# hillerlab/GenomeAlignmentTools

Measured on AMD Instinct MI355X. Metric: aligned Gbases scored/sec, chainNet -rescore hg38-mm10, 1/2/4/8 MI355X, higher is better.
Workload: dtype int64; 1 GPU; chainNet -rescore end to end (bin/chainNet), C5 whole genome; generator=gac_synth c5, seed=1234, scale=1, t_seqs=455, q_seqs=66, chains=4999999, blocks=116489921, input_aligned_bases=4660467906, netted_chains=4701362, netted_aligned_bases=4397257687, parallelism=chromosome-side shards x1

## Files before the change

### genomealignmenttools_amd/csrc/host/gac_net.c

```c
#define _GNU_SOURCE
#include "gac_host.h"

#include <immintrin.h>
#include <sched.h>
#include <stdint.h>
#include <sys/mman.h>
#include <pthread.h>
#include <stdatomic.h>
#include <math.h>
#include <stdarg.h>
#include <stdio.h>
#include <time.h>
#include <stdlib.h>
#include <string.h>

#define BIGNUM 0x3fffffff

typedef struct ngap ngap;
typedef struct nfill nfill;

struct ngap {
    int start, end, o_start, o_end;
    nfill *fill_head;
    nfill **fills;
    int n_fills;
    ngap *next;
    nfill *pfill;
    int32_t pidx;
};

struct nfill {
    int start, end, o_start, o_end;
    int32_t chain;
    int32_t ali;
    ngap **gaps;
    int n_gaps;
    int32_t full;
    nfill *next;
    int64_t ord;
    ngap *pgap;
    int32_t pidx, level;
    int32_t wb0, wn;
};

typedef struct nchrom {
    const char *name;
    int size;
    ngap *root;
    int32_t sroot;
    int32_t height;
} nchrom;

typedef struct arena {
    char **blocks;
    size_t *sizes;
    size_t n, cap, used, bsize;
} arena;

#define ARENA_BLOCK ((size_t)32 << 20)
#define ARENA_ALIGN ((size_t)2 << 20)

static char *arena_map(size_t bs) {
    size_t len = bs + ARENA_ALIGN;
    char *m = mmap(NULL, len, PROT_READ | PROT_WRITE, MAP_PRIVATE | MAP_ANONYMOUS, -1, 0);
    if (m == MAP_FAILED) {
        fprintf(stderr, "gac_net: out of memory mapping %zu bytes\n", bs);
        abort();
    }
    char *p = (char *)(((uintptr_t)m + ARENA_ALIGN - 1) & ~(uintptr_t)(ARENA_ALIGN - 1));
    if (p > m)
        munmap(m, (size_t)(p - m));
    if (p + bs < m + len)
        munmap(p + bs, (size_t)(m + len - (p + bs)));
#ifdef MADV_HUGEPAGE
    madvise(p, bs, MADV_HUGEPAGE);
#endif
    return p;
}

static void *arena_alloc(arena *a, size_t sz) {
    sz = (sz + 15) & ~(size_t)15;
    if (a->n == 0 || a->used + sz > a->bsize) {
        if (a->n == a->cap) {
            a->cap = a->cap ? a->cap * 2 : 64;
            a->blocks = realloc(a->blocks, a->cap * sizeof(char *));
            a->sizes = realloc(a->sizes, a->cap * sizeof(size_t));
        }
        size_t bs = sz > ARENA_BLOCK ? (sz + ARENA_ALIGN - 1) & ~(ARENA_ALIGN - 1) : ARENA_BLOCK;
        a->blocks[a->n] = arena_map(bs);
        a->sizes[a->n++] = bs;
        a->bsize = bs;
        a->used = 0;
    }
    char *p = a->blocks[a->n - 1] + a->used;
    a->used += sz;
    if (a->used + 512 <= a->bsize)
        __builtin_prefetch(p + sz + 384, 1, 3);
    return p;
}

static int g_free_madv = -1;

static void arena_free(arena *a) {
    for (size_t i = 0; i < a->n && g_free_madv == 1; ++i)
        madvise(a->blocks[i], a->sizes[i], MADV_DONTNEED);
    for (size_t i = 0; i < a->n; ++i)
        munmap(a->blocks[i], a->sizes[i]);
    free(a->blocks);
    free(a->sizes);
    memset(a, 0, sizeof(*a));
}

typedef struct nwork {
    arena ar;
    struct sleaf *lf;
    int32_t lf_n, lf_cap, lf_free;
    struct snode *in;
    int32_t in_n, in_cap, in_free;
    struct sitem *q, *it, *cmb;
    int64_t q_n, q_cap, it_n, it_cap, cmb_cap;
    int32_t *rs, *re, *ros, *roe, *ro;
    int64_t r_cap;
    struct nfill **sf;
    int64_t sf_cap;
    char pad[64];
} nwork;

struct gac_net {
    gac_net_input in;
    gac_net_opts opt;
    int64_t n_netted;
    nchrom *chroms[2];
    int32_t n_chroms[2];
    nwork *w;
    int n_w;
    int64_t *chain_ali;
    nfill **order[2];
    int64_t n_order[2];
    int64_t *pord[2];
    int pord_ok[2];
    pthread_mutex_t pord_mu;
    int64_t *top[2];
    int64_t n_top[2];
    int32_t *nlen[2];
    int sides;
    int lookahead;
    atomic_int free_next;
// ... 370 lines not shown
        sleaf *L = &w->lf[y];
        for (int k = lo; k < hi; ++k) {
            L->start[k - lo] = cb[k].start;
            L->end[k - lo] = cb[k].end;
            L->gap[k - lo] = cb[k].gap;
        }
        L->n = hi - lo;
        if (p > 0) {
            L->prev = prev;
            w->lf[prev].next = y;
        }
        prev = y;
        nk[p] = spkey(cb[lo].start, cb[lo].end);
        nc[p] = y;
    }
    w->lf[prev].next = after;
    if (after >= 0)
        w->lf[after].prev = prev;
    sp_inner_insert(w, c, pn, pi, H - 1, nk + 1, nc + 1, parts - 1);
    free(nk);
    free(nc);
}

static ngap *gap_new(nwork *n, int s, int e, int os, int oe) {
    ngap *g = arena_alloc(&n->ar, sizeof(ngap));
    g->start = s;
    g->end = e;
    g->o_start = os;
    g->o_end = oe;
    return g;
}

static int strictly_inside(const gac_net *n, int min_start, int max_end, int start, int end) {
    return min_start < start && start + n->opt.min_space <= end && end < max_end;
}

static void it_push(nwork *w, int32_t s, int32_t e, ngap *g) {
    if (w->it_n == w->it_cap) {
        w->it_cap = w->it_cap ? w->it_cap * 2 : 1024;
        w->it = realloc(w->it, (size_t)w->it_cap * sizeof(sitem));
    }
    w->it[w->it_n++] = (sitem){s, e, g};
}


static void add_chain_side(const gac_net *net, nwork *n, nchrom *c, int32_t chain, int nb,
                           const int32_t *s, const int32_t *e, const int32_t *gos,
                           const int32_t *goe, const int32_t *os, int inv, int oflip, int cstart,
                           int cend, int boff) {
    sp_query(n, c, cstart, cend, s, e, nb);
    const int64_t nsp = n->q_n;
    for (int64_t si = 0; si < nsp; ++si)
        __builtin_prefetch(&n->q[si].gap->fill_head, 1);
    int k = 0;
    for (int64_t si = 0; si < nsp; ++si) {
        const int sstart = n->q[si].start, send = n->q[si].end;
        ngap *sgap = n->q[si].gap;
        while (k + 1 < nb && s[k + 1] <= sstart)
            ++k;
        int start = BIGNUM, end = -BIGNUM, zero = 0;
        int fs = BIGNUM, fe = -BIGNUM, omin = BIGNUM, omax = -BIGNUM;
        int wfirst = -1, wlast = -2;
        int64_t ali = 0;
        for (int b = k; b < nb; ++b) {
            const int b0 = s[b], b1 = e[b];
            if (b1 <= sstart)
                continue;
            if (b0 >= send)
                break;
            if (wfirst < 0)
                wfirst = b;
            wlast = b;
            const int cs = b0 < sstart ? sstart : b0, ce = b1 > send ? send : b1;
            if (start > cs)
                start = cs;
            if (end < ce)
                end = ce;
            ali += ce - cs;
            if (ce > cs) {
                const int o0 = inv ? os[b] + (b1 - ce) : os[b] + (cs - b0);
                const int o1 = inv ? os[b] + (b1 - cs) : os[b] + (ce - b0);
                if (fs > cs) fs = cs;
                if (fe < ce) fe = ce;
                if (omin > o0) omin = o0;
                if (omax < o1) omax = o1;
            } else {
                zero = 1;
            }
        }
        if (end < 0 || end - start < net->opt.min_fill)
            continue;
        nfill *f = arena_alloc(&n->ar, sizeof(nfill));
        f->start = start;
        f->end = end;
        f->chain = chain;
        f->ali = (int32_t)ali;
        if (zero) {
            fs = BIGNUM, fe = -BIGNUM, omin = BIGNUM, omax = -BIGNUM;
            for (int b = k; b < nb; ++b) {
                const int bs = s[b], be = e[b];
                if (be <= start)
                    continue;
                if (bs >= end)
                    break;
                const int cs = bs < start ? start : bs, ce = be > end ? end : be;
                const int o0 = inv ? os[b] + (be - ce) : os[b] + (cs - bs);
                const int o1 = inv ? os[b] + (be - cs) : os[b] + (ce - bs);
                if (fs > cs) fs = cs;
                if (fe < ce) fe = ce;
                if (omin > o0) omin = o0;
                if (omax < o1) omax = o1;
            }
        }
        {
            if (oflip >= 0) {
                const int t = omin;
                omin = oflip - omax;
                omax = oflip - t;
            }
            f->start = fs;
            f->end = fe;
            f->o_start = omin;
            f->o_end = omax;
            f->full = fs <= cstart && fe >= cend;
        }
        if (boff >= 0) {
            if (zero) {
                wfirst = k;
                while (wfirst < nb && e[wfirst] <= fs)
                    ++wfirst;
                wlast = wfirst - 1;
                while (wlast + 1 < nb && s[wlast + 1] < fe)
                    ++wlast;
            }
            f->wb0 = boff + (wfirst < 0 ? 0 : wfirst);
            f->wn = wfirst < 0 ? 0 : wlast - wfirst + 1;
        }
        nfill *h = __atomic_load_n(&sgap->fill_head, __ATOMIC_RELAXED);
        do
            f->next = h;
        while (!__atomic_compare_exchange_n(&sgap->fill_head, &h, f, 1, __ATOMIC_RELEASE,
                                            __ATOMIC_RELAXED));
        n->it_n = 0;
        if (start - sstart >= net->opt.min_space)
            it_push(n, sstart, start, sgap);
        const int64_t g0 = n->it_n;
        for (int b = k; b + 1 < nb; ++b) {
            int gs = e[b], ge = s[b + 1];
            if (ge >= send)
                break;
            if (strictly_inside(net, sstart, send, gs, ge))
                it_push(n, gs, ge, gap_new(n, gs, ge, gos[b], goe[b]));
        }
        f->n_gaps = (int)(n->it_n - g0);
        f->gaps = f->n_gaps ? arena_alloc(&n->ar, f->n_gaps * sizeof(ngap *)) : NULL;
        for (int i = 0; i < f->n_gaps; ++i)
            f->gaps[i] = n->it[g0 + i].gap;
        if (send - end >= net->opt.min_space)
            it_push(n, end, send, sgap);
        sp_replace(n, c, sstart, send, n->it, (int)n->it_n);
    }
}

static void ensure_rev(nwork *n, int64_t nb) {
    if (nb > n->r_cap) {
        n->r_cap = nb * 2;
        n->rs = realloc(n->rs, n->r_cap * 4);
        n->re = realloc(n->re, n->r_cap * 4);
        n->ros = realloc(n->ros, n->r_cap * 4);
        n->roe = realloc(n->roe, n->r_cap * 4);
        n->ro = realloc(n->ro, n->r_cap * 4);
    }
}

static int is_haplotype(const char *name) {
    return strstr(name, "_hap") != NULL || strstr(name, "_alt") != NULL;
}

typedef struct crec {
    int64_t boff;
// ... 105 lines not shown
}

static int cmp_fill(const void *a, const void *b) {
    const nfill *x = *(nfill *const *)a, *y = *(nfill *const *)b;
    return (x->start > y->start) - (x->start < y->start);
}

typedef struct fin_ctx {
    gac_net *n;
    nwork *w;
    int side;
    nfill **ord;
    int64_t n_ord, cap;
} fin_ctx;

static void finish_gap(fin_ctx *x, ngap *g);

static void finish_fill(fin_ctx *x, nfill *f) {
    if (x->n_ord == x->cap) {
        x->cap = x->cap ? x->cap * 2 : 256;
        x->ord = realloc(x->ord, (size_t)x->cap * sizeof(nfill *));
    }
    x->ord[x->n_ord++] = f;
    for (int i = 0; i < f->n_gaps; ++i) {
        f->gaps[i]->pfill = f;
        f->gaps[i]->pidx = i;
    }
    for (int i = 0; i < f->n_gaps; ++i)
        finish_gap(x, f->gaps[i]);
}

static void sort_gap_fills(nwork *w, ngap *g) {
    if (!g->fill_head) {
        g->n_fills = 0;
        g->fills = NULL;
        return;
    }
    int cnt = 0;
    for (nfill *f = g->fill_head; f; f = f->next) {
        if (cnt == w->sf_cap) {
            w->sf_cap = w->sf_cap ? 2 * w->sf_cap : 4096;
            w->sf = realloc(w->sf, (size_t)w->sf_cap * sizeof(nfill *));
        }
        w->sf[cnt++] = f;
    }
    g->n_fills = cnt;
    g->fills = arena_alloc(&w->ar, cnt * sizeof(nfill *));
    copy_fill(g->fills, w->sf, cnt);
    const int32_t level = g->pfill ? g->pfill->level + 1 : 0;
    if (cnt <= 16) {
        for (int i = 1; i < cnt; ++i) {
            nfill *v = g->fills[i];
            int j = i - 1;
            while (j >= 0 && g->fills[j]->start > v->start) {
                g->fills[j + 1] = g->fills[j];
                --j;
            }
            g->fills[j + 1] = v;
        }
    } else {
        qsort(g->fills, g->n_fills, sizeof(nfill *), cmp_fill);
    }
    for (int i = 0; i < cnt; ++i) {
        g->fills[i]->pgap = g;
        g->fills[i]->pidx = i;
        g->fills[i]->level = level;
    }
}

static void finish_gap(fin_ctx *x, ngap *g) {
    sort_gap_fills(x->w, g);
    for (int i = 0; i < g->n_fills; ++i)
        finish_fill(x, g->fills[i]);
}

static void *free_worker(void *arg) {
    gac_net *n = arg;
    for (;;) {
        int i = atomic_fetch_add(&n->free_next, 1);
        if (i >= n->n_w)
            return NULL;
        nwork *w = &n->w[i];
        arena_free(&w->ar);
        free(w->lf);
        free(w->in);
        free(w->q);
        free(w->it);
        free(w->cmb);
        free(w->rs);
        free(w->re);
        free(w->ros);
        free(w->roe);
        free(w->ro);
        free(w->sf);
    }
}
// ... 156 lines not shown

typedef struct sk_item {
    nfill *f;
    ngap *g;
    int64_t cnt;
} sk_item;

typedef struct skel {
    sk_item *it;
    int64_t n, cap;
} skel;

static void sk_push(skel *k, nfill *f, ngap *g) {
    if (k->n == k->cap) {
        k->cap = k->cap ? k->cap * 2 : 256;
        k->it = realloc(k->it, (size_t)k->cap * sizeof(sk_item));
    }
    k->it[k->n++] = (sk_item){f, g, 0};
}

static void skel_fill(nwork *w, skel *k, nfill *f) {
    sk_push(k, f, NULL);
    for (int i = 0; i < f->n_gaps; ++i) {
        f->gaps[i]->pfill = f;
        f->gaps[i]->pidx = i;
    }
    for (int i = 0; i < f->n_gaps; ++i) {
        ngap *g = f->gaps[i];
        if (f->level < SKEL_DEPTH) {
            sort_gap_fills(w, g);
            for (int j = 0; j < g->n_fills; ++j)
                skel_fill(w, k, g->fills[j]);
        } else if (g->fill_head) {
            sk_push(k, NULL, g);
        } else {
            g->n_fills = 0;
            g->fills = NULL;
        }
    }
}

typedef struct ispan {
    nfill **src;
    int64_t pos, cnt;
    int side;
} ispan;

typedef struct splice_job {
    gac_net *n;
    ispan *sp;
    int64_t nspan;
    _Atomic int64_t next;
} splice_job;

static void *splice_thread(void *arg) {
    splice_job *J = arg;
    for (;;) {
        const int64_t a = atomic_fetch_add(&J->next, 4096);
        if (a >= J->nspan)
            return NULL;
// ... 17 lines not shown
    sk_item **gi;
    int64_t n_gi, per;
    fin_ctx *x;
    int64_t ntask;
    _Atomic int64_t next;
    _Atomic int wid;
} fin_job;

static void *fin_thread(void *arg) {
    fin_job *F = arg;
    gac_net *n = F->n;
    nwork *w = &n->w[atomic_fetch_add(&F->wid, 1)];
    if (F->phase == 0) {
        const int64_t nc = n->n_chroms[GAC_T] + (int64_t)n->n_chroms[GAC_Q];
        for (;;) {
            const int64_t k = atomic_fetch_add(&F->next, 1);
            if (k >= nc)
                break;
            const int side = k < n->n_chroms[GAC_T] ? GAC_T : GAC_Q;
            nchrom *c = &n->chroms[side][side == GAC_T ? k : k - n->n_chroms[GAC_T]];
            if (!c->root)
                continue;
            sort_gap_fills(w, c->root);
            for (int j = 0; j < c->root->n_fills; ++j)
                skel_fill(w, &F->sk[k], c->root->fills[j]);
        }
        return NULL;
    }
    for (;;) {
        const int64_t k = atomic_fetch_add(&F->next, 1);
        if (k >= F->ntask)
            break;
        fin_ctx *x = &F->x[k];
        x->n = n;
        x->w = w;
        const int64_t a = k * F->per, b = a + F->per < F->n_gi ? a + F->per : F->n_gi;
        for (int64_t i = a; i < b; ++i) {
            const int64_t before = x->n_ord;
            finish_gap(x, F->gi[i]->g);
            F->gi[i]->cnt = x->n_ord - before;
        }
    }
    return NULL;
}

typedef struct net_task {
    int side;
    int32_t chrom;
// ... 240 lines not shown
    }
    free(bin);
    int64_t *rw = calloc((size_t)nc + 1, 8), mx = 0;
    for (int64_t i = 0; i < rest; ++i) {
        const int cs = t->recs[B->m + i].s, ce = t->recs[B->m + i].e;
        const int64_t a = upper_bound32(cuts, nc, cs), b = upper_bound32(cuts, nc, ce > cs ? ce - 1 : cs);
        for (int64_t r = a; r <= b; ++r)
            rw[r] += chain_work_in(cs, ce, t->recs[B->m + i].nb, r ? cuts[r - 1] : 0,
                                   r < nc ? cuts[r] : size);
    }
    for (int32_t r = 0; r <= nc; ++r)
        mx = rw[r] > mx ? rw[r] : mx;
    free(rw);
    *pmax = mx;
    *ptot = tot;
    return nc + 1;
}

static double mono_s(void);

static void big_prefix(gac_net *n, nwork *w, big_net *B, int nthreads) {
    net_task *t = B->t;
    nchrom *c = &n->chroms[t->side][t->chrom];
    c->root = gap_new(w, 0, c->size, 0, 0);
    c->root->pidx = t->chrom;
    sp_init(w, c, 0, c->size, c->root);
    const int32_t want = 4 * nthreads;
    int32_t *cuts = malloc((size_t)want * 4);
    B->t_start = mono_s();
    int64_t m = t->n < 8 ? t->n : 8, done = 0;
    sitem *sp = NULL;
    int64_t nsp = 0;
    int32_t nreg = 1;
    double t_add = 0, t_cut = 0, t0 = mono_s();
    const double t_gather = t0 - B->t_start;
    for (;;) {
        double ta = mono_s();
        net_chains(n, w, t->side, t->recs + done, m - done, c, INT32_MIN, INT32_MAX);
        done = m;
        double tb = mono_s();
        t_add += tb - ta;
        B->m = m;
        free(sp);
        sp = sp_all(w, c, &nsp);
        int64_t mx, tot;
        nreg = place_cuts(n, B, sp, nsp, want, c->size, cuts, &mx, &tot);
        t_cut += mono_s() - tb;
        if (m >= t->n || mx * nthreads <= tot * 5 / 4 || m >= t->n / 4)
// ... 60 lines not shown
    net_task *task;
    int64_t ntask;
    big_net *big;
    int32_t nbig;
    region **rq;
    int64_t nrq;
    _Atomic int64_t next, rnext, rpub;
    pthread_mutex_t rmu;
    _Atomic int ready;
    _Atomic int wid;
    _Atomic int32_t bnext, bdone;
    int nthreads;
    double t0;
    double prefix_s;
} net_job;

static int region_cmp(const void *a, const void *b) {
    const region *x = *(region *const *)a, *y = *(region *const *)b;
    return (x->work < y->work) - (x->work > y->work);
}

static void net_small(gac_net *n, nwork *w, const net_task *t) {
    nchrom *c = &n->chroms[t->side][t->chrom];
    c->root = gap_new(w, 0, c->size, 0, 0);
    c->root->pidx = t->chrom;
    sp_init(w, c, 0, c->size, c->root);
    net_chains(n, w, t->side, t->recs, t->n, c, INT32_MIN, INT32_MAX);
}

static double mono_s(void) {
    struct timespec t;
    clock_gettime(CLOCK_MONOTONIC, &t);
    return t.tv_sec + 1e-9 * t.tv_nsec;
}

static void *net_thread(void *arg) {
    net_job *J = arg;
    const int id = atomic_fetch_add(&J->wid, 1);
    nwork *w = &J->n->w[id];
    for (;;) {
        const int32_t b = atomic_fetch_add(&J->bnext, 1);
        if (b >= J->nbig)
            break;
        big_prefix(J->n, w, &J->big[b], J->nthreads);
        big_net *B = &J->big[b];
        region **tmp = malloc((size_t)(B->n_reg ? B->n_reg : 1) * sizeof(region *));
        for (int32_t r = 0; r < B->n_reg; ++r)
            tmp[r] = &B->reg[r];
// ... 179 lines not shown
        return gac_fail(GAC_E_ARG, "gac_net_build_sides: bad side mask %d", sides);
    return net_build(in, opt, sides, NULL, NULL, out);
}

int gac_net_build_subset(const gac_net_input *in, const gac_net_opts *opt, const uint8_t *t_keep,
                         const uint8_t *q_keep, gac_net **out) {
    gac_clear_error();
    if (!in || !opt || !out || !t_keep || !q_keep)
        return gac_fail(GAC_E_ARG, "gac_net_build_subset: NULL argument");
    return net_build(in, opt, (1 << GAC_T) | (1 << GAC_Q), t_keep, q_keep, out);
}

static int net_build(const gac_net_input *in, const gac_net_opts *opt, int sides,
                     const uint8_t *t_keep, const uint8_t *q_keep, gac_net **out) {
    *out = NULL;
    gac_net *n = calloc(1, sizeof(*n));
    if (n)
        pthread_mutex_init(&n->pord_mu, NULL);
    n->in = *in;
    n->opt = *opt;
    n->sides = sides;
    n->n_w = gac_host_threads();
    n->w = calloc((size_t)n->n_w, sizeof(nwork));
    for (int k = 0; k < n->n_w; ++k) {
        n->w[k].lf_free = -1;
        n->w[k].in_free = -1;
    }
    struct timespec t_set0, t_set1;
    clock_gettime(CLOCK_MONOTONIC, &t_set0);
    double last = -1;
    int64_t i;
    for (i = 0; i < in->n_chains; ++i) {
        const double sc = in->score[i];
        if (last >= 0 && sc > last) {
            gac_net_free(n);
            return gac_fail(GAC_E_FORMAT, "input must be sorted in order of score");
        }
        last = sc;
        if (sc < opt->min_score)
            break;
        if (in->t_seq[i] < 0 || in->t_seq[i] >= in->n_tseq || in->q_seq[i] < 0 ||
            in->q_seq[i] >= in->n_qseq) {
            gac_net_free(n);
            return gac_fail(GAC_E_ARG, "chain %lld: sequence index out of range", (long long)i);
        }
    }
    const int64_t nn = i;
    int32_t nt = in->n_tseq, nq = in->n_qseq;
    int64_t *toff, *qoff;
// ... 132 lines not shown
            for (int64_t i = 0; i < F.sk[k].n; ++i)
                tot[side] += F.sk[k].it[i].g ? F.sk[k].it[i].cnt : 1;
        }
        for (int side = 0; side < 2; ++side) {
            n->order[side] = malloc((size_t)(tot[side] ? tot[side] : 1) * sizeof(nfill *));
            n->n_order[side] = 0;
        }
        int64_t nspan = 0;
        for (int64_t k = 0; k < nc; ++k)
            nspan += F.sk[k].n;
        splice_job SJ = {n, malloc((size_t)(nspan ? nspan : 1) * sizeof(ispan)), nspan, 0};
        for (int side = 0; side < 2; ++side) {
            n->top[side] = malloc((size_t)(nspan ? nspan : 1) * sizeof(int64_t));
            n->n_top[side] = 0;
        }
        {
            int64_t gidx = 0, used = 0, m = 0;
            for (int64_t k = 0; k < nc; ++k) {
                const int side = k < n->n_chroms[GAC_T] ? GAC_T : GAC_Q;
                for (int64_t i = 0; i < F.sk[k].n; ++i) {
                    sk_item *it = &F.sk[k].it[i];
                    if (!it->g) {
                        SJ.sp[m++] = (ispan){&it->f, n->n_order[side], 1, side};
                        if (it->f->level == 0)
                            n->top[side][n->n_top[side]++] = n->n_order[side];
                        ++n->n_order[side];
                        continue;
                    }
                    const fin_ctx *x = &F.x[gidx / F.per];
                    if (gidx % F.per == 0)
                        used = 0;
                    SJ.sp[m++] = (ispan){x->ord + used, n->n_order[side], it->cnt, side};
                    n->n_order[side] += it->cnt;
                    used += it->cnt;
                    ++gidx;
                }
            }
        }
        atomic_init(&SJ.next, 0);
        gac_run_threads(n->n_w, splice_thread, &SJ);
        free(SJ.sp);
        for (int64_t k = 0; k < nc; ++k)
            free(F.sk[k].it);
        for (int64_t k = 0; k < F.ntask; ++k)
            free(F.x[k].ord);
        free(F.sk);
        free(F.gi);
        struct timespec t_b;
        clock_gettime(CLOCK_MONOTONIC, &t_b);
        if (getenv("GAC_TIMING"))
            fprintf(stderr, "[gac_net_build] finishNet skeletons %.3f s, subtrees %.3f s, index %.3f s (%lld gap subtrees in %lld chunks)\n",
                    (t_a.tv_sec - t_fin0.tv_sec) + 1e-9 * (t_a.tv_nsec - t_fin0.tv_nsec),
                    (t_sp.tv_sec - t_a.tv_sec) + 1e-9 * (t_sp.tv_nsec - t_a.tv_nsec),
                    (t_b.tv_sec - t_sp.tv_sec) + 1e-9 * (t_b.tv_nsec - t_sp.tv_nsec), (long long)F.n_gi,
                    (long long)F.ntask);
        free(F.x);
    }
    clock_gettime(CLOCK_MONOTONIC, &t_fin1);
    if (getenv("GAC_TIMING")) {
        size_t sp_bytes = 0, ar_bytes = 0;
        for (int i = 0; i < n->n_w; ++i) {
            sp_bytes += (size_t)n->w[i].lf_cap * sizeof(sleaf) + (size_t)n->w[i].in_cap * sizeof(snode);
            for (size_t k = 0; k < n->w[i].ar.n; ++k)
                ar_bytes += n->w[i].ar.sizes[k];
        }
        fprintf(stderr, "[gac_net_build] finishNet %.3f s (space index %.0f MB, fill/gap arenas %.0f MB)\n",
                (t_fin1.tv_sec - t_fin0.tv_sec) + 1e-9 * (t_fin1.tv_nsec - t_fin0.tv_nsec),
                sp_bytes / 1e6, ar_bytes / 1e6);
    }
    space_release(n);
    for (int side = 0; side < 2; ++side) {
        const int32_t ns = side == GAC_T ? in->n_tseq : in->n_qseq;
        const char *const *nm = side == GAC_T ? in->t_names : in->q_names;
        n->nlen[side] = malloc((size_t)(ns > 0 ? ns : 1) * sizeof(int32_t));
        for (int32_t k = 0; k < ns; ++k)
            n->nlen[side][k] = (int32_t)strlen(nm[k]);
    }
    n->chain_ali = malloc((size_t)(in->n_chains ? in->n_chains : 1) * sizeof(int64_t));
    {
        ca_job A = {in, n->chain_ali, 0};
        atomic_init(&A.next, 0);
        gac_run_threads(gac_host_threads(), chain_ali_thread, &A);
    }
    *out = n;
    return GAC_OK;
}

int64_t gac_net_netted(const gac_net *n) { return n ? n->n_netted : -1; }

int64_t gac_net_fill_count(const gac_net *n, int side) {
    if (!n || (side != GAC_T && side != GAC_Q))
// ... 6 lines not shown
typedef struct gf_job {
    const gac_net *n;
    int side;
    int32_t *chain, *start, *end, *ali;
    uint8_t *flags;
    int64_t per;
    _Atomic int64_t next;
    int32_t *wb0, *wn;
    int64_t *po;
} gf_job;

static void *fills_thread(void *arg) {
    gf_job *J = arg;
    const gac_net *n = J->n;
    const int side = J->side;
    for (;;) {
        const int64_t a = atomic_fetch_add(&J->next, 1) * J->per;
        if (a >= n->n_order[side])
            break;
        const int64_t b = a + J->per < n->n_order[side] ? a + J->per : n->n_order[side];
        for (int64_t i = a; i < b; ++i) {
            const nfill *f = n->order[side][i];
            const int64_t c = f->chain;
            const int full = f->full;
            const int sz = full ? full_size(n, c) : f->ali;
            if (J->chain)
                J->chain[i] = (int32_t)c;
            if (J->start)
                J->start[i] = f->start;
            if (J->end)
                J->end[i] = f->end;
            if (J->ali)
                J->ali[i] = sz;
            if (J->flags)
                J->flags[i] = (uint8_t)(full ? 0 : 1);
            if (J->wb0)
                J->wb0[i] = f->wb0;
            if (J->wn)
                J->wn[i] = f->wn;
        }
    }
    return NULL;
}

static int64_t next_top_level(const gac_net *n, int side, int64_t i) {
    if (n->top[side]) {
        const int64_t *t = n->top[side];
        int64_t lo = 0, hi = n->n_top[side];
        while (lo < hi) {
            const int64_t mid = (lo + hi) >> 1;
            if (t[mid] < i)
                lo = mid + 1;
            else
                hi = mid;
        }
        return lo < n->n_top[side] ? t[lo] : n->n_order[side];
    }
    if (__atomic_load_n(&n->pord_ok[side], __ATOMIC_ACQUIRE)) {
        const int64_t *po = n->pord[side];
        while (i < n->n_order[side] && po[i] >= 0)
            ++i;
        return i;
    }
    while (i < n->n_order[side] && n->order[side][i]->pgap->pfill)
        ++i;
    return i;
}

static void *visible_thread(void *arg) {
    gf_job *J = arg;
    const gac_net *n = J->n;
    const int side = J->side;
    const int64_t nf = n->n_order[side];
    for (;;) {
        const int64_t r = atomic_fetch_add(&J->next, 1);
        if (r * J->per >= nf)
            break;
        const int64_t a = next_top_level(n, side, r * J->per);
        const int64_t b = next_top_level(n, side, (r + 1) * J->per < nf ? (r + 1) * J->per : nf);
        int64_t *po = J->po;
        for (int64_t i = a; i < b; ++i) {
            const nfill *pf = n->order[side][i]->pgap->pfill;
            if (po)
                po[i] = pf ? pf->ord : -1;
            const int sz = J->ali ? J->ali[i] : 0;
            if ((!pf || (J->flags[pf->ord] & 2)) && sz >= n->opt.min_fill)
                J->flags[i] |= 2;
        }
    }
    return NULL;
}

int gac_net_get_fills(const gac_net *n, int side, int32_t *chain, int32_t *start, int32_t *end,
                      int32_t *ali, uint8_t *flags) {
    if (!n || (side != GAC_T && side != GAC_Q))
        return gac_fail(GAC_E_ARG, "gac_net_get_fills: bad argument");
    if (!(n->sides & (1 << side)))
        return gac_fail(GAC_E_STATE, "gac_net_get_fills: side %d was not netted", side);
    const int nt = gac_host_threads();
    const int64_t nf = n->n_order[side];
    gf_job J = {n, side, chain, start, end, ali, flags, nf / (8 * (int64_t)nt) + 1, 0, NULL, NULL};
    atomic_init(&J.next, 0);
    const int64_t nrun = (nf + J.per - 1) / J.per;
    gac_mark("get_fills: fills");
    gac_run_threads(nt < nrun ? nt : (int)(nrun ? nrun : 1), fills_thread, &J);
// ... 54 lines not shown
    const gac_net *n = J->n;
    const int side = J->side;
    const int64_t nf = n->n_order[side];
    for (;;) {
        const int64_t r = atomic_fetch_add(&J->next, 1);
        if (r >= J->nrun)
            break;
        rw_run *R = &J->runs[r];
        if (J->phase == 1) {
            if (R->n) {
                memcpy(J->out + J->off[r], R->w, (size_t)R->n * sizeof(gac_window));
                memcpy(J->opos + J->off[r], R->pos, (size_t)R->n * sizeof(int64_t));
            }
            free(R->w);
            free(R->pos);
            continue;
        }
        const int64_t a = next_top_level(n, side, r * J->per);
        const int64_t b = next_top_level(n, side, (r + 1) * J->per < nf ? (r + 1) * J->per : nf);
        for (int64_t i = a; i < b; ++i) {
            if (i + 16 < b)
                __builtin_prefetch(n->order[side][i + 16]);
            const nfill *f = n->order[side][i];
            const nfill *pf = f->pgap->pfill;
            if (J->po)
                J->po[i] = pf ? pf->ord : -1;
            const int sz = f->full ? full_size(n, f->chain) : f->ali;
            const uint8_t v = (!pf || J->vis[pf->ord]) && sz >= n->opt.min_fill;
            J->vis[i] = v;
            if (!v || f->full)
                continue;
            if (R->n == R->cap) {
                R->cap = R->cap ? 2 * R->cap : 4096;
                R->w = realloc(R->w, (size_t)R->cap * sizeof(gac_window));
                R->pos = realloc(R->pos, (size_t)R->cap * sizeof(int64_t));
            }
            R->w[R->n] = (gac_window){(int32_t)f->chain, f->start, f->end, f->wb0, f->wn};
            R->pos[R->n++] = i;
        }
    }
    return NULL;
}

int gac_net_rescore_windows(const gac_net *n, int side, gac_window **windows, int64_t **pos,
                            int64_t *count) {
    if (!n || side != GAC_T || !windows || !pos || !count)
        return gac_fail(GAC_E_ARG, "gac_net_rescore_windows: bad argument (target side only)");
    if (!(n->sides & (1 << side)))
        return gac_fail(GAC_E_STATE, "gac_net_rescore_windows: side %d was not netted", side);
    const int nt = gac_host_threads();
    const int64_t nf = n->n_order[side];
    gac_net *nm = (gac_net *)n;
    pthread_mutex_lock(&nm->pord_mu);
// ... 147 lines not shown
    p = put_spaces(p, depth);
    p = put_str(p, "gap ");
    p = put_int(p, g->start);
    *p++ = ' ';
    p = put_int(p, g->end - g->start);
    *p++ = ' ';
    p = put_str(p, ochrom);
    *p++ = ' ';
    *p++ = in->q_strand[c] ? '-' : '+';
    *p++ = ' ';
    p = put_int(p, g->o_start);
    *p++ = ' ';
    p = put_int(p, g->o_end - g->o_start);
    *p++ = '\n';
    w->o->n += (size_t)(p - buf);
}

static int fill_info(const gac_net *n, int side, const int64_t *tscore, const nfill *f,
                     double *score_out, int *sub_out) {
    const gac_net_input *in = &n->in;
    const int64_t c = f->chain;
    int sub;
    double score;
    if (f->full) {
        score = in->score[c];
        sub = full_size(n, c);
    } else {
        sub = f->ali;
        if (side == GAC_T && tscore == k_deferred) {
            score = 1;
        } else if (side == GAC_T && tscore) {
            double r = (double)tscore[f->ord];
            score = r <= 0 ? 1 : r;
        } else {
            score = in->score[c] * sub / full_size(n, c);
        }
    }
    *score_out = score;
    *sub_out = sub;
    return score >= n->opt.min_score && sub >= n->opt.min_fill;
}

static void put_fill_line(const wctx *w, const nfill *f, int depth, double score, int sub) {
    const gac_net_input *in = &w->n->in;
    const int64_t c = f->chain;
    const char *ochrom = w->side == GAC_Q ? in->t_names[in->t_seq[c]] : in->q_names[in->q_seq[c]];
    const int olen = w->side == GAC_Q ? w->n->nlen[GAC_T][in->t_seq[c]] : w->n->nlen[GAC_Q][in->q_seq[c]];
    const int deferred = w->marks && w->side == GAC_T && !f->full;
    if (olen > 400 || depth > 400 || !(score > -1e300 && score < 1e300)) {
        gac_obuf_printf(w->o, "%*sfill %d %d %s %c %d %d id %d score ", depth, "", f->start,
                  f->end - f->start, ochrom, in->q_strand[c] ? '-' : '+', f->o_start,
                  f->o_end - f->o_start, in->id[c]);
        if (deferred) {
            wmarks *m = w->marks;
            if (m->n == m->cap) {
                m->cap = m->cap ? 2 * m->cap : 256;
                m->m = realloc(m->m, (size_t)m->cap * sizeof(wmark));
            }
            m->m[m->n++] = (wmark){(int64_t)w->o->n, f->ord};
        } else {
            gac_obuf_printf(w->o, "%1.0f", score);
        }
        gac_obuf_printf(w->o, " ali %d\n", sub);
        return;
    }
    char *const buf = gac_obuf_reserve(w->o, 512 + 400 + 400), *p = buf;
    p = put_spaces(p, depth);
    p = put_str(p, "fill ");
    p = put_int(p, f->start);
    *p++ = ' ';
    p = put_int(p, f->end - f->start);
// ... 25 lines not shown
}

typedef struct wjob {
    const gac_net *n;
    int side;
    const int64_t *tscore;
    wmarks *marks;
    const nfill *const *ord;
    int64_t nf, per;
    double *score;
    int32_t *sub;
    uint8_t *show;
    uint8_t *more;
    uint8_t *reached;
    uint16_t *lvl;
    int32_t *pix;
    _Atomic int deep;
    _Atomic int64_t next;
} wjob;

static int gap_prints_fill(const wjob *J, const ngap *g) {
    if (g->n_fills == 0)
        return 0;
    const int64_t o = g->fills[0]->ord;
    return J->show[o] || J->more[o];
}

static void write_segment(const wjob *J, wctx *w, int64_t i) {
    const nfill *f = J->ord[i];
    if (!f->pgap->pfill && f->pidx == 0) {
        const nchrom *c = &J->n->chroms[J->side][f->pgap->pidx];
        gac_obuf_printf(w->o, "net %s %d\n", c->name, c->size);
    }
    if (!J->reached[i])
        return;
    put_fill_line(w, f, 2 * f->level + 1, J->score[i], J->sub[i]);
    const nfill *cur = f;
    int g0 = 0;
    for (;;) {
        for (int gi = g0; gi < cur->n_gaps; ++gi) {
            const ngap *g = cur->gaps[gi];
            put_gap_line(w, cur, g, 2 * cur->level + 2);
            if (gap_prints_fill(J, g))
                return;
        }
        if (J->more[cur->ord])
            return;
        const ngap *pg = cur->pgap;
        if (!pg->pfill)
            return;
        g0 = pg->pidx + 1;
        cur = pg->pfill;
    }
}

static void write_run(gac_obuf *o, int64_t r, void *arg) {
    wjob *J = arg;
    const int64_t a = r * J->per;
    const int64_t b = a + J->per < J->nf ? a + J->per : J->nf;
    wctx w = {J->n, o, J->side, J->tscore, 0, NULL, J->marks ? &J->marks[r] : NULL};
    const gac_net_input *in = &J->n->in;
    for (int64_t i = a; i < b; ++i) {
        if (i + 16 < b)
            __builtin_prefetch(J->ord[i + 16]);
        if (i + 8 < b) {
            const nfill *f = J->ord[i + 8];
            __builtin_prefetch(f->gaps);
            __builtin_prefetch(&in->q_seq[f->chain]);
            __builtin_prefetch(&in->q_strand[f->chain]);
            __builtin_prefetch(&in->id[f->chain]);
            __builtin_prefetch(&in->t_seq[f->chain]);
        }
        if (i + 4 < b) {
            const nfill *f = J->ord[i + 4];
            for (int k = 0; k < f->n_gaps && k < 4; ++k)
                __builtin_prefetch(f->gaps[k]);
        }
        write_segment(J, &w, i);
    }
}

static void *winfo_thread(void *arg) {
    wjob *J = arg;
    for (;;) {
        const int64_t a = atomic_fetch_add(&J->next, 4096);
        if (a >= J->nf)
            break;
        const int64_t b = a + 4096 < J->nf ? a + 4096 : J->nf;
        for (int64_t i = a; i < b; ++i) {
            if (i + 16 < b)
                __builtin_prefetch(J->ord[i + 16]);
            if (i + 8 < b) {
                const int64_t c = J->ord[i + 8]->chain;
                __builtin_prefetch(&J->n->in.score[c]);
                __builtin_prefetch(&J->n->chain_ali[c]);
            }
            J->show[i] = (uint8_t)fill_info(J->n, J->side, J->tscore, J->ord[i], &J->score[i],
                                            &J->sub[i]);
            const int32_t L = J->ord[i]->level;
            J->lvl[i] = (uint16_t)(L < 65535 ? L : 65535);
            J->pix[i] = J->ord[i]->pidx;
            if (L >= 65535)
                atomic_store(&J->deep, 1);
        }
    }
    return NULL;
}

static void mark_more(wjob *J, const ngap *g) {
    uint8_t any = 0;
    for (int k = g->n_fills - 1; k >= 0; --k) {
        const int64_t o = g->fills[k]->ord;
        J->more[o] = any;
        any |= J->show[o];
    }
}

static void *wmore_thread(void *arg) {
    wjob *J = arg;
    for (;;) {
        const int64_t a = atomic_fetch_add(&J->next, 4096);
        if (a >= J->nf)
            break;
        const int64_t b = a + 4096 < J->nf ? a + 4096 : J->nf;
        for (int64_t i = a; i < b; ++i) {
            if (i + 16 < b)
                __builtin_prefetch(J->ord[i + 16]);
            if (i + 8 < b) {
                const nfill *p = J->ord[i + 8];
                for (int k = 0; k < p->n_gaps && k < 4; ++k)
                    __builtin_prefetch(p->gaps[k]);
            }
            const nfill *f = J->ord[i];
            for (int k = 0; k < f->n_gaps; ++k)
                mark_more(J, f->gaps[k]);
        }
    }
    return NULL;
}

static int net_write_f(const gac_net *n, int side, const int64_t *tscores, FILE *f,
                       const char *const *meta, int32_t n_meta, void (*on_formatted)(void *),
                       void *harg);

static void *wmore_lvl_thread(void *arg) {
    wjob *J = arg;
    const int64_t per = J->nf / (8 * (int64_t)gac_host_threads()) + 1;
    for (;;) {
        const int64_t r = atomic_fetch_add(&J->next, 1);
        if (r * per >= J->nf)
            return NULL;
        const int64_t a = next_top_level(J->n, J->side, r * per);
        const int64_t b = next_top_level(J->n, J->side, (r + 1) * per < J->nf ? (r + 1) * per : J->nf);
        int32_t pbuf[256], *prev = pbuf;
        uint8_t abuf[256], *acc = abuf;
        int cap = 256;
        for (int k = 0; k < cap; ++k)
            prev[k] = INT32_MIN;
// ... 51 lines not shown
        }
        if (!atomic_load(&J->deep)) {
            int64_t stk[256], *last = stk;
            int cap = 256;
            for (int64_t i = a; i < b; ++i) {
                const int L = J->lvl[i];
                if (L >= cap) {
                    const int nc = L + 256;
                    int64_t *q = malloc((size_t)nc * sizeof(int64_t));
                    memcpy(q, last, (size_t)cap * sizeof(int64_t));
                    if (last != stk)
                        free(last);
                    last = q;
                    cap = nc;
                }
                last[L] = i;
                J->reached[i] = J->show[i] && (L == 0 || J->reached[last[L - 1]]);
            }
            if (last != stk)
                free(last);
            continue;
        }
        for (int64_t i = a; i < b; ++i) {
            const nfill *pf = J->ord[i]->pgap->pfill;
            J->reached[i] = J->show[i] && (!pf || J->reached[pf->ord]);
        }
    }
}

int gac_net_write(const gac_net *n, int side, const int64_t *tscores, const char *path,
                  const char *const *meta, int32_t n_meta) {
    return gac_net_write_ex(n, side, tscores, path, meta, n_meta, NULL, NULL);
}

int gac_net_write_ex(const gac_net *n, int side, const int64_t *tscores, const char *path,
                     const char *const *meta, int32_t n_meta, void (*on_formatted)(void *),
                     void *harg) {
    if (!n || !path || (side != GAC_T && side != GAC_Q))
        return gac_fail(GAC_E_ARG, "gac_net_write: bad argument");
    if (!(n->sides & (1 << side)))
        return gac_fail(GAC_E_STATE, "gac_net_write: side %d was not netted", side);
    FILE *f;
    int close_it = 1;
    if (strcmp(path, "stdout") == 0) {
        f = stdout;
        close_it = 0;
    } else {
// ... 31 lines not shown
    J->n = n;
    J->side = side;
    J->tscore = side == GAC_T ? tscore : NULL;
    J->ord = (const nfill *const *)n->order[side];
    J->nf = nf;
    const size_t m = (size_t)(nf ? nf : 1);
    J->score = malloc(m * sizeof(double));
    J->sub = malloc(m * sizeof(int32_t));
    J->show = malloc(m);
    J->more = malloc(m);
    J->reached = malloc(m);
    J->lvl = malloc(m * sizeof(uint16_t));
    J->pix = malloc(m * sizeof(int32_t));
    atomic_init(&J->deep, 0);
    const int nt = gac_host_threads();
    atomic_init(&J->next, 0);
    gac_run_threads(nt, winfo_thread, J);
    gac_mark("flags: info done");
    atomic_store(&J->next, 0);
    gac_run_threads(nt, atomic_load(&J->deep) ? wmore_thread : wmore_lvl_thread, J);
    gac_mark("flags: more done");
    for (int32_t k = 0; k < n->n_chroms[side]; ++k) {
        const nchrom *c = &n->chroms[side][k];
        if (c->root && c->root->fill_head)
            mark_more(J, c->root);
    }
    gac_mark("flags: roots done");
    atomic_store(&J->next, 0);
    gac_run_threads(nt, wreached_thread, J);
    gac_mark("flags: reached done");
    J->per = nf / (64 * (int64_t)nt) + 1;
}

static void wjob_free_flags(wjob *J) {
    free(J->score);
    free(J->sub);
    free(J->show);
    free(J->more);
    free(J->reached);
    free(J->lvl);
    free(J->pix);
    J->lvl = NULL;
    J->pix = NULL;
    J->score = NULL;
    J->sub = NULL;
    J->show = J->more = J->reached = NULL;
}
// ... 143 lines not shown
```

Before: 3.128 Gbases/s.

## Pack fills and their gaps into contiguous cache-line groups

Shrinks the fill record to one 64-byte cache line and the gap record to 32 bytes. Each fill's gaps are now allocated inline right after it, replacing separately allocated gaps and a pointer array. Parent links become index arithmetic, level and full share one field, and single-fill gaps store the fill inline instead of allocating an array. The aim is fewer allocations and pointer chases and a smaller memory footprint in net building, finishing and writing. In exchange it reserves a worst-case gap count per fill, aborts if that bound is exceeded, and adds an env-tunable arena block size.

```diff
diff --git a/genomealignmenttools_amd/csrc/host/gac_net.c b/genomealignmenttools_amd/csrc/host/gac_net.c
--- a/genomealignmenttools_amd/csrc/host/gac_net.c
+++ b/genomealignmenttools_amd/csrc/host/gac_net.c
@@ -19,13 +19,16 @@
 typedef struct ngap ngap;
 typedef struct nfill nfill;
 
+#define GAP_ROOT INT32_MIN
+
 struct ngap {
     int start, end, o_start, o_end;
-    nfill *fill_head;
-    nfill **fills;
-    int n_fills;
-    ngap *next;
-    nfill *pfill;
+    union {
+        nfill *fill_head;
+        nfill **fills;
+        nfill *one;
+    } u;
+    int32_t n_fills;
     int32_t pidx;
 };
 
@@ -33,15 +36,32 @@
     int start, end, o_start, o_end;
     int32_t chain;
     int32_t ali;
-    ngap **gaps;
-    int n_gaps;
-    int32_t full;
-    nfill *next;
+    int32_t n_gaps;
+    int32_t pidx;
     int64_t ord;
-    ngap *pgap;
-    int32_t pidx, level;
+    union {
+        nfill *next;
+        ngap *pgap;
+    } u;
     int32_t wb0, wn;
-};
+    uint32_t lvfull;
+    int32_t pad;
+} __attribute__((aligned(64)));
+
+_Static_assert(sizeof(nfill) == 64, "a fill is one cache line");
+_Static_assert(_Alignof(nfill) == 64, "a fill starts a cache line");
+_Static_assert(sizeof(ngap) == 32, "two gaps per cache line");
+_Static_assert(sizeof(nfill) % sizeof(ngap) == 0, "gaps follow their fill without padding");
+
+static inline ngap *fill_gap(const nfill *f, int i) { return (ngap *)(f + 1) + i; }
+static inline int32_t fill_level(const nfill *f) { return (int32_t)(f->lvfull >> 1); }
+static inline int fill_full(const nfill *f) { return (int)(f->lvfull & 1); }
+static inline nfill *gap_parent(const ngap *g) {
+    return g->pidx < 0 ? NULL : (nfill *)((char *)(g - g->pidx) - sizeof(nfill));
+}
+static inline nfill *const *gap_fills(const ngap *g) {
+    return g->n_fills == 1 ? (nfill *const *)&g->u.one : (nfill *const *)g->u.fills;
+}
 
 typedef struct nchrom {
     const char *name;
@@ -55,12 +75,26 @@
     char **blocks;
     size_t *sizes;
     size_t n, cap, used, bsize;
+    size_t block;
 } arena;
 
 #define ARENA_BLOCK ((size_t)32 << 20)
 #define ARENA_ALIGN ((size_t)2 << 20)
 
+static size_t arena_block_size(void) {
+    const char *e = getenv("GAC_NET_ARENA_BLOCK");
+    return e && atoll(e) > 0 ? ((size_t)atoll(e) + 63) & ~(size_t)63 : ARENA_BLOCK;
+}
+
 static char *arena_map(size_t bs) {
+    if (bs < ARENA_ALIGN) {
+        char *m = mmap(NULL, bs, PROT_READ | PROT_WRITE, MAP_PRIVATE | MAP_ANONYMOUS, -1, 0);
+        if (m == MAP_FAILED) {
+            fprintf(stderr, "gac_net: out of memory mapping %zu bytes\n", bs);
+            abort();
+        }
+        return m;
+    }
     size_t len = bs + ARENA_ALIGN;
     char *m = mmap(NULL, len, PROT_READ | PROT_WRITE, MAP_PRIVATE | MAP_ANONYMOUS, -1, 0);
     if (m == MAP_FAILED) {
@@ -78,25 +112,49 @@
     return p;
 }
 
+static void arena_grow(arena *a, size_t sz) {
+    if (a->n == a->cap) {
+        a->cap = a->cap ? a->cap * 2 : 64;
+        a->blocks = realloc(a->blocks, a->cap * sizeof(char *));
+        a->sizes = realloc(a->sizes, a->cap * sizeof(size_t));
+    }
+    const size_t block = a->block ? a->block : ARENA_BLOCK;
+    const size_t q = block < ARENA_ALIGN ? block : ARENA_ALIGN;
+    const size_t bs = sz > block ? (sz + q - 1) / q * q : block;
+    a->blocks[a->n] = arena_map(bs);
+    a->sizes[a->n++] = bs;
+    a->bsize = bs;
+    a->used = 0;
+}
+
 static void *arena_alloc(arena *a, size_t sz) {
     sz = (sz + 15) & ~(size_t)15;
-    if (a->n == 0 || a->used + sz > a->bsize) {
-        if (a->n == a->cap) {
-            a->cap = a->cap ? a->cap * 2 : 64;
-            a->blocks = realloc(a->blocks, a->cap * sizeof(char *));
-            a->sizes = realloc(a->sizes, a->cap * sizeof(size_t));
-        }
-        size_t bs = sz > ARENA_BLOCK ? (sz + ARENA_ALIGN - 1) & ~(ARENA_ALIGN - 1) : ARENA_BLOCK;
-        a->blocks[a->n] = arena_map(bs);
-        a->sizes[a->n++] = bs;
-        a->bsize = bs;
-        a->used = 0;
-    }
+    if (a->n == 0 || a->used + sz > a->bsize)
+        arena_grow(a, sz);
     char *p = a->blocks[a->n - 1] + a->used;
     a->used += sz;
     if (a->used + 512 <= a->bsize)
         __builtin_prefetch(p + sz + 384, 1, 3);
     return p;
+}
+
+static nfill *arena_reserve_group(arena *a, int max_gaps) {
+    const size_t sz = sizeof(nfill) + (size_t)max_gaps * sizeof(ngap);
+    size_t u = (a->used + 63) & ~(size_t)63;
+    if (a->n == 0 || u + sz > a->bsize) {
+        arena_grow(a, sz);
+        u = 0;
+    }
+    a->used = u;
+    return (nfill *)(a->blocks[a->n - 1] + u);
+}
+
+static void arena_commit_group(arena *a, int n_gaps) {
+    const size_t sz = (sizeof(nfill) + (size_t)n_gaps * sizeof(ngap) + 63) & ~(size_t)63;
+    char *p = a->blocks[a->n - 1] + a->used;
+    a->used += sz;
+    if (a->used + 512 <= a->bsize)
+        __builtin_prefetch(p + sz + 384, 1, 3);
 }
 
 static int g_free_madv = -1;
@@ -123,6 +181,7 @@
     int64_t r_cap;
     struct nfill **sf;
     int64_t sf_cap;
+    int64_t n_fill, n_gap;
     char pad[64];
 } nwork;
 
@@ -539,12 +598,14 @@
     free(nc);
 }
 
-static ngap *gap_new(nwork *n, int s, int e, int os, int oe) {
+static ngap *root_gap_new(nwork *n, int size, int32_t chrom) {
     ngap *g = arena_alloc(&n->ar, sizeof(ngap));
-    g->start = s;
-    g->end = e;
-    g->o_start = os;
-    g->o_end = oe;
+    g->start = 0;
+    g->end = size;
+    g->o_start = 0;
+    g->o_end = 0;
+    g->pidx = GAP_ROOT | chrom;
+    ++n->n_gap;
     return g;
 }
 
@@ -568,7 +629,7 @@
     sp_query(n, c, cstart, cend, s, e, nb);
     const int64_t nsp = n->q_n;
     for (int64_t si = 0; si < nsp; ++si)
-        __builtin_prefetch(&n->q[si].gap->fill_head, 1);
+        __builtin_prefetch(&n->q[si].gap->u.fill_head, 1);
     int k = 0;
     for (int64_t si = 0; si < nsp; ++si) {
         const int sstart = n->q[si].start, send = n->q[si].end;
@@ -607,9 +668,8 @@
         }
         if (end < 0 || end - start < net->opt.min_fill)
             continue;
-        nfill *f = arena_alloc(&n->ar, sizeof(nfill));
-        f->start = start;
-        f->end = end;
+        const int max_gaps = wlast - wfirst;
+        nfill *f = arena_reserve_group(&n->ar, max_gaps);
         f->chain = chain;
         f->ali = (int32_t)ali;
         if (zero) {
@@ -639,7 +699,7 @@
             f->end = fe;
             f->o_start = omin;
             f->o_end = omax;
-            f->full = fs <= cstart && fe >= cend;
+            f->lvfull = fs <= cstart && fe >= cend;
         }
         if (boff >= 0) {
             if (zero) {
@@ -653,26 +713,37 @@
             f->wb0 = boff + (wfirst < 0 ? 0 : wfirst);
             f->wn = wfirst < 0 ? 0 : wlast - wfirst + 1;
         }
-        nfill *h = __atomic_load_n(&sgap->fill_head, __ATOMIC_RELAXED);
+        nfill *h = __atomic_load_n(&sgap->u.fill_head, __ATOMIC_RELAXED);
         do
-            f->next = h;
-        while (!__atomic_compare_exchange_n(&sgap->fill_head, &h, f, 1, __ATOMIC_RELEASE,
+            f->u.next = h;
+        while (!__atomic_compare_exchange_n(&sgap->u.fill_head, &h, f, 1, __ATOMIC_RELEASE,
                                             __ATOMIC_RELAXED));
         n->it_n = 0;
         if (start - sstart >= net->opt.min_space)
             it_push(n, sstart, start, sgap);
-        const int64_t g0 = n->it_n;
+        int ng = 0;
         for (int b = k; b + 1 < nb; ++b) {
             int gs = e[b], ge = s[b + 1];
             if (ge >= send)
                 break;
-            if (strictly_inside(net, sstart, send, gs, ge))
-                it_push(n, gs, ge, gap_new(n, gs, ge, gos[b], goe[b]));
-        }
-        f->n_gaps = (int)(n->it_n - g0);
-        f->gaps = f->n_gaps ? arena_alloc(&n->ar, f->n_gaps * sizeof(ngap *)) : NULL;
-        for (int i = 0; i < f->n_gaps; ++i)
-            f->gaps[i] = n->it[g0 + i].gap;
+            if (strictly_inside(net, sstart, send, gs, ge)) {
+                if (ng == max_gaps) {
+                    fprintf(stderr, "gac_net: more gaps than a fill's group holds\n");
+                    abort();
+                }
+                ngap *g = fill_gap(f, ng);
+                g->start = gs;
+                g->end = ge;
+                g->o_start = gos[b];
+                g->o_end = goe[b];
+                g->pidx = ng++;
+                it_push(n, gs, ge, g);
+            }
+        }
+        f->n_gaps = ng;
+        arena_commit_group(&n->ar, ng);
+        ++n->n_fill;
+        n->n_gap += ng;
         if (send - end >= net->opt.min_space)
             it_push(n, end, send, sgap);
         sp_replace(n, c, sstart, send, n->it, (int)n->it_n);
@@ -824,56 +895,60 @@
         x->ord = realloc(x->ord, (size_t)x->cap * sizeof(nfill *));
     }
     x->ord[x->n_ord++] = f;
-    for (int i = 0; i < f->n_gaps; ++i) {
-        f->gaps[i]->pfill = f;
-        f->gaps[i]->pidx = i;
-    }
     for (int i = 0; i < f->n_gaps; ++i)
-        finish_gap(x, f->gaps[i]);
+        finish_gap(x, fill_gap(f, i));
 }
 
 static void sort_gap_fills(nwork *w, ngap *g) {
-    if (!g->fill_head) {
-        g->n_fills = 0;
-        g->fills = NULL;
+    nfill *const head = g->u.fill_head;
+    if (!head)
         return;
+    const nfill *const pf = gap_parent(g);
+    const uint32_t level2 = pf ? (uint32_t)(fill_level(pf) + 1) << 1 : 0;
+    if (!head->u.next) {
+        g->n_fills = 1;
+        head->u.pgap = g;
+        head->pidx = 0;
+        head->lvfull = level2 | (head->lvfull & 1);
+        return;
     }
     int cnt = 0;
-    for (nfill *f = g->fill_head; f; f = f->next) {
+    for (nfill *f = head; f; f = f->u.next) {
         if (cnt == w->sf_cap) {
             w->sf_cap = w->sf_cap ? 2 * w->sf_cap : 4096;
             w->sf = realloc(w->sf, (size_t)w->sf_cap * sizeof(nfill *));
         }
         w->sf[cnt++] = f;
     }
+    nfill **fills = arena_alloc(&w->ar, cnt * sizeof(nfill *));
     g->n_fills = cnt;
-    g->fills = arena_alloc(&w->ar, cnt * sizeof(nfill *));
-    copy_fill(g->fills, w->sf, cnt);
-    const int32_t level = g->pfill ? g->pfill->level + 1 : 0;
+    g->u.fills = fills;
+    copy_fill(fills, w->sf, cnt);
     if (cnt <= 16) {
         for (int i = 1; i < cnt; ++i) {
-            nfill *v = g->fills[i];
+            nfill *v = fills[i];
             int j = i - 1;
-            while (j >= 0 && g->fills[j]->start > v->start) {
-                g->fills[j + 1] = g->fills[j];
+            while (j >= 0 && fills[j]->start > v->start) {
+                fills[j + 1] = fills[j];
                 --j;
             }
-            g->fills[j + 1] = v;
+            fills[j + 1] = v;
         }
     } else {
-        qsort(g->fills, g->n_fills, sizeof(nfill *), cmp_fill);
+        qsort(fills, cnt, sizeof(nfill *), cmp_fill);
     }
     for (int i = 0; i < cnt; ++i) {
-        g->fills[i]->pgap = g;
-        g->fills[i]->pidx = i;
-        g->fills[i]->level = level;
+        fills[i]->u.pgap = g;
+        fills[i]->pidx = i;
+        fills[i]->lvfull = level2 | (fills[i]->lvfull & 1);
     }
 }
 
 static void finish_gap(fin_ctx *x, ngap *g) {
     sort_gap_fills(x->w, g);
+    nfill *const *fills = gap_fills(g);
     for (int i = 0; i < g->n_fills; ++i)
-        finish_fill(x, g->fills[i]);
+        finish_fill(x, fills[i]);
 }
 
 static void *free_worker(void *arg) {
@@ -1076,20 +1151,14 @@
 static void skel_fill(nwork *w, skel *k, nfill *f) {
     sk_push(k, f, NULL);
     for (int i = 0; i < f->n_gaps; ++i) {
-        f->gaps[i]->pfill = f;
-        f->gaps[i]->pidx = i;
-    }
-    for (int i = 0; i < f->n_gaps; ++i) {
-        ngap *g = f->gaps[i];
-        if (f->level < SKEL_DEPTH) {
+        ngap *g = fill_gap(f, i);
+        if (fill_level(f) < SKEL_DEPTH) {
             sort_gap_fills(w, g);
+            nfill *const *fills = gap_fills(g);
             for (int j = 0; j < g->n_fills; ++j)
-                skel_fill(w, k, g->fills[j]);
-        } else if (g->fill_head) {
+                skel_fill(w, k, fills[j]);
+        } else if (g->u.fill_head) {
             sk_push(k, NULL, g);
-        } else {
-            g->n_fills = 0;
-            g->fills = NULL;
         }
     }
 }
@@ -1153,8 +1222,9 @@
             if (!c->root)
                 continue;
             sort_gap_fills(w, c->root);
+            nfill *const *fills = gap_fills(c->root);
             for (int j = 0; j < c->root->n_fills; ++j)
-                skel_fill(w, &F->sk[k], c->root->fills[j]);
+                skel_fill(w, &F->sk[k], fills[j]);
         }
         return NULL;
     }
@@ -1441,8 +1511,7 @@
 static void big_prefix(gac_net *n, nwork *w, big_net *B, int nthreads) {
     net_task *t = B->t;
     nchrom *c = &n->chroms[t->side][t->chrom];
-    c->root = gap_new(w, 0, c->size, 0, 0);
-    c->root->pidx = t->chrom;
+    c->root = root_gap_new(w, c->size, t->chrom);
     sp_init(w, c, 0, c->size, c->root);
     const int32_t want = 4 * nthreads;
     int32_t *cuts = malloc((size_t)want * 4);
@@ -1549,8 +1618,7 @@
 
 static void net_small(gac_net *n, nwork *w, const net_task *t) {
     nchrom *c = &n->chroms[t->side][t->chrom];
-    c->root = gap_new(w, 0, c->size, 0, 0);
-    c->root->pidx = t->chrom;
+    c->root = root_gap_new(w, c->size, t->chrom);
     sp_init(w, c, 0, c->size, c->root);
     net_chains(n, w, t->side, t->recs, t->n, c, INT32_MIN, INT32_MAX);
 }
@@ -1776,9 +1844,11 @@
     n->sides = sides;
     n->n_w = gac_host_threads();
     n->w = calloc((size_t)n->n_w, sizeof(nwork));
+    const size_t ablock = arena_block_size();
     for (int k = 0; k < n->n_w; ++k) {
         n->w[k].lf_free = -1;
         n->w[k].in_free = -1;
+        n->w[k].ar.block = ablock;
     }
     struct timespec t_set0, t_set1;
     clock_gettime(CLOCK_MONOTONIC, &t_set0);
@@ -1957,7 +2027,7 @@
                     sk_item *it = &F.sk[k].it[i];
                     if (!it->g) {
                         SJ.sp[m++] = (ispan){&it->f, n->n_order[side], 1, side};
-                        if (it->f->level == 0)
+                        if (fill_level(it->f) == 0)
                             n->top[side][n->n_top[side]++] = n->n_order[side];
                         ++n->n_order[side];
                         continue;
@@ -1994,14 +2064,17 @@
     clock_gettime(CLOCK_MONOTONIC, &t_fin1);
     if (getenv("GAC_TIMING")) {
         size_t sp_bytes = 0, ar_bytes = 0;
+        long long fills = 0, gaps = 0;
         for (int i = 0; i < n->n_w; ++i) {
+            fills += n->w[i].n_fill;
+            gaps += n->w[i].n_gap;
             sp_bytes += (size_t)n->w[i].lf_cap * sizeof(sleaf) + (size_t)n->w[i].in_cap * sizeof(snode);
             for (size_t k = 0; k < n->w[i].ar.n; ++k)
                 ar_bytes += n->w[i].ar.sizes[k];
         }
-        fprintf(stderr, "[gac_net_build] finishNet %.3f s (space index %.0f MB, fill/gap arenas %.0f MB)\n",
+        fprintf(stderr, "[gac_net_build] finishNet %.3f s (space index %.0f MB, fill/gap arenas %.0f MB: %lld fills of %zu bytes, %lld gaps of %zu bytes)\n",
                 (t_fin1.tv_sec - t_fin0.tv_sec) + 1e-9 * (t_fin1.tv_nsec - t_fin0.tv_nsec),
-                sp_bytes / 1e6, ar_bytes / 1e6);
+                sp_bytes / 1e6, ar_bytes / 1e6, fills, sizeof(nfill), gaps, sizeof(ngap));
     }
     space_release(n);
     for (int side = 0; side < 2; ++side) {
@@ -2054,7 +2127,7 @@
         for (int64_t i = a; i < b; ++i) {
             const nfill *f = n->order[side][i];
             const int64_t c = f->chain;
-            const int full = f->full;
+            const int full = fill_full(f);
             const int sz = full ? full_size(n, c) : f->ali;
             if (J->chain)
                 J->chain[i] = (int32_t)c;
@@ -2094,7 +2167,7 @@
             ++i;
         return i;
     }
-    while (i < n->n_order[side] && n->order[side][i]->pgap->pfill)
+    while (i < n->n_order[side] && gap_parent(n->order[side][i]->u.pgap))
         ++i;
     return i;
 }
@@ -2112,7 +2185,7 @@
         const int64_t b = next_top_level(n, side, (r + 1) * J->per < nf ? (r + 1) * J->per : nf);
         int64_t *po = J->po;
         for (int64_t i = a; i < b; ++i) {
-            const nfill *pf = n->order[side][i]->pgap->pfill;
+            const nfill *pf = gap_parent(n->order[side][i]->u.pgap);
             if (po)
                 po[i] = pf ? pf->ord : -1;
             const int sz = J->ali ? J->ali[i] : 0;
@@ -2213,13 +2286,13 @@
             if (i + 16 < b)
                 __builtin_prefetch(n->order[side][i + 16]);
             const nfill *f = n->order[side][i];
-            const nfill *pf = f->pgap->pfill;
+            const nfill *pf = gap_parent(f->u.pgap);
             if (J->po)
                 J->po[i] = pf ? pf->ord : -1;
-            const int sz = f->full ? full_size(n, f->chain) : f->ali;
+            const int sz = fill_full(f) ? full_size(n, f->chain) : f->ali;
             const uint8_t v = (!pf || J->vis[pf->ord]) && sz >= n->opt.min_fill;
             J->vis[i] = v;
-            if (!v || f->full)
+            if (!v || fill_full(f))
                 continue;
             if (R->n == R->cap) {
                 R->cap = R->cap ? 2 * R->cap : 4096;
@@ -2413,7 +2486,7 @@
     const int64_t c = f->chain;
     int sub;
     double score;
-    if (f->full) {
+    if (fill_full(f)) {
         score = in->score[c];
         sub = full_size(n, c);
     } else {
@@ -2437,7 +2510,7 @@
     const int64_t c = f->chain;
     const char *ochrom = w->side == GAC_Q ? in->t_names[in->t_seq[c]] : in->q_names[in->q_seq[c]];
     const int olen = w->side == GAC_Q ? w->n->nlen[GAC_T][in->t_seq[c]] : w->n->nlen[GAC_Q][in->q_seq[c]];
-    const int deferred = w->marks && w->side == GAC_T && !f->full;
+    const int deferred = w->marks && w->side == GAC_T && !fill_full(f);
     if (olen > 400 || depth > 400 || !(score > -1e300 && score < 1e300)) {
         gac_obuf_printf(w->o, "%*sfill %d %d %s %c %d %d id %d score ", depth, "", f->start,
                   f->end - f->start, ochrom, in->q_strand[c] ? '-' : '+', f->o_start,
@@ -2509,35 +2582,35 @@
 static int gap_prints_fill(const wjob *J, const ngap *g) {
     if (g->n_fills == 0)
         return 0;
-    const int64_t o = g->fills[0]->ord;
+    const int64_t o = gap_fills(g)[0]->ord;
     return J->show[o] || J->more[o];
 }
 
 static void write_segment(const wjob *J, wctx *w, int64_t i) {
     const nfill *f = J->ord[i];
-    if (!f->pgap->pfill && f->pidx == 0) {
-        const nchrom *c = &J->n->chroms[J->side][f->pgap->pidx];
+    if (f->u.pgap->pidx < 0 && f->pidx == 0) {
+        const nchrom *c = &J->n->chroms[J->side][f->u.pgap->pidx & INT32_MAX];
         gac_obuf_printf(w->o, "net %s %d\n", c->name, c->size);
     }
     if (!J->reached[i])
         return;
-    put_fill_line(w, f, 2 * f->level + 1, J->score[i], J->sub[i]);
+    put_fill_line(w, f, 2 * fill_level(f) + 1, J->score[i], J->sub[i]);
     const nfill *cur = f;
     int g0 = 0;
     for (;;) {
         for (int gi = g0; gi < cur->n_gaps; ++gi) {
-            const ngap *g = cur->gaps[gi];
-            put_gap_line(w, cur, g, 2 * cur->level + 2);
+            const ngap *g = fill_gap(cur, gi);
+            put_gap_line(w, cur, g, 2 * fill_level(cur) + 2);
             if (gap_prints_fill(J, g))
                 return;
         }
         if (J->more[cur->ord])
             return;
-        const ngap *pg = cur->pgap;
-        if (!pg->pfill)
+        const ngap *pg = cur->u.pgap;
+        if (pg->pidx < 0)
             return;
         g0 = pg->pidx + 1;
-        cur = pg->pfill;
+        cur = gap_parent(pg);
     }
 }
 
@@ -2552,7 +2625,6 @@
             __builtin_prefetch(J->ord[i + 16]);
         if (i + 8 < b) {
             const nfill *f = J->ord[i + 8];
-            __builtin_prefetch(f->gaps);
             __builtin_prefetch(&in->q_seq[f->chain]);
             __builtin_prefetch(&in->q_strand[f->chain]);
             __builtin_prefetch(&in->id[f->chain]);
@@ -2560,8 +2632,8 @@
         }
         if (i + 4 < b) {
             const nfill *f = J->ord[i + 4];
-            for (int k = 0; k < f->n_gaps && k < 4; ++k)
-                __builtin_prefetch(f->gaps[k]);
+            for (int k = 0; k < f->n_gaps && k < 4; k += 2)
+                __builtin_prefetch(fill_gap(f, k));
         }
         write_segment(J, &w, i);
     }
@@ -2584,7 +2656,7 @@
             }
             J->show[i] = (uint8_t)fill_info(J->n, J->side, J->tscore, J->ord[i], &J->score[i],
                                             &J->sub[i]);
-            const int32_t L = J->ord[i]->level;
+            const int32_t L = fill_level(J->ord[i]);
             J->lvl[i] = (uint16_t)(L < 65535 ? L : 65535);
             J->pix[i] = J->ord[i]->pidx;
             if (L >= 65535)
@@ -2596,8 +2668,9 @@
 
 static void mark_more(wjob *J, const ngap *g) {
     uint8_t any = 0;
+    nfill *const *fills = gap_fills(g);
     for (int k = g->n_fills - 1; k >= 0; --k) {
-        const int64_t o = g->fills[k]->ord;
+        const int64_t o = fills[k]->ord;
         J->more[o] = any;
         any |= J->show[o];
     }
@@ -2615,12 +2688,12 @@
                 __builtin_prefetch(J->ord[i + 16]);
             if (i + 8 < b) {
                 const nfill *p = J->ord[i + 8];
-                for (int k = 0; k < p->n_gaps && k < 4; ++k)
-                    __builtin_prefetch(p->gaps[k]);
+                for (int k = 0; k < p->n_gaps && k < 4; k += 2)
+                    __builtin_prefetch(fill_gap(p, k));
             }
             const nfill *f = J->ord[i];
             for (int k = 0; k < f->n_gaps; ++k)
-                mark_more(J, f->gaps[k]);
+                mark_more(J, fill_gap(f, k));
         }
     }
     return NULL;
@@ -2718,7 +2791,7 @@
             continue;
         }
         for (int64_t i = a; i < b; ++i) {
-            const nfill *pf = J->ord[i]->pgap->pfill;
+            const nfill *pf = gap_parent(J->ord[i]->u.pgap);
             J->reached[i] = J->show[i] && (!pf || J->reached[pf->ord]);
         }
     }
@@ -2796,7 +2869,7 @@
     gac_mark("flags: more done");
     for (int32_t k = 0; k < n->n_chroms[side]; ++k) {
         const nchrom *c = &n->chroms[side][k];
-        if (c->root && c->root->fill_head)
+        if (c->root && c->root->n_fills)
             mark_more(J, c->root);
     }
     gac_mark("flags: roots done");
```

Result: faster. 3.420 Gbases/s, median of 6 (+9.3%).
